# floe/backscrub

Measured on AMD Instinct MI355X. Metric: composited frames/sec at 640×480 (batch), 1/2/4/8 MI355X + mask IoU vs CPU ref, higher is better.
Workload: dtype f32 (network) / u8 (image kernels); 1 GPU; BASELINE configs[1]: batch=256 640x480 frames, segm_lite_v681.tflite; moving scene: ring of 4 batches, a new one every step; 1 step = prep+network+decode+mask+blend, inputs resident in HBM; streams_per_gpu=256, library=bsx 0.1 (HIP gfx950, f32 NHWC)

## Files before the change

backscrub_amd/csrc/gen_seg.cpp:

```cpp
#include "gen_seg.hpp"

#include <cstdarg>
#include <cstdio>

namespace bsx {
namespace {

const char kSegSource[] =
#include "seg_rtc_src.inc"
    ;

}

std::string seg_constants_text(const SegPlan& sp, const char* pre) {
  std::string out;
  auto P = [&](const char* fmt, ...) {
    char buf[1024];
    va_list ap;
    va_start(ap, fmt);
    vsnprintf(buf, sizeof buf, fmt, ap);
    va_end(ap);
    out += buf;
  };
  auto conv = [&](const char* n, const SegConvW& c) { P("  t.%s.w_off = %lldll; t.%s.b_off = %lldll; t.%s.Cin = %d; t.%s.Cout = %d; t.%s.cout_pad = %d; t.%s.act = %d;\n", n, c.w_off, n, c.b_off, n, c.Cin, n, c.Cout, n, c.cout_pad, n, c.act); };
  auto dw = [&](const char* n, const SegDwW& c) { P("  t.%s.w_off = %lldll; t.%s.b_off = %lldll; t.%s.C = %d; t.%s.act = %d;\n", n, c.w_off, n, c.b_off, n, c.C, n, c.act); };
  auto gate = [&](const char* n, const SegGate& g_) {
    P("  t.%s.n_parts = %d; t.%s.sum_parts = %d; t.%s.n_fc = %d; t.%s.timing_skip = %d;\n", n, g_.n_parts, n, g_.sum_parts, n, g_.n_fc, n, g_.timing_skip);
    for (int i = 0; i < 2; i++) {
      P("  t.%s.part[%d].off = %lldll; t.%s.part[%d].n = %d; t.%s.part[%d].C = %d; t.%s.part[%d].hw = (float)%.9g;\n", n, i, g_.part[i].off, n, i, g_.part[i].n, n, i, g_.part[i].C, n, i, (double)g_.part[i].hw);
      P("  t.%s.fc[%d].w_off = %lldll; t.%s.fc[%d].b_off = %lldll; t.%s.fc[%d].Cin = %d; t.%s.fc[%d].Cout = %d; t.%s.fc[%d].act = %d;\n", n, i, g_.fc[i].w_off, n, i, g_.fc[i].b_off, n, i, g_.fc[i].Cin, n, i,
              g_.fc[i].Cout, n, i, g_.fc[i].act);
    }
  };
  auto end = [&](int dbg_skip) { if (dbg_skip) P("  t.dbg_skip = %d;\n", dbg_skip); P("  return t; }();\n"); };
  const SegHead& H = sp.head; const SegK2& K2 = sp.k2; const SegK3& K3 = sp.k3; const SegTail& T = sp.tail;
  P("// segment descriptors of the loaded graph as constants (gen_seg.cpp: seg_constants_text)\nconstexpr SegHead %sHEAD = [] { SegHead t{};\n", pre);
  P("  t.H0 = %d; t.W0 = %d; t.H1 = %d; t.W1 = %d; t.H2 = %d; t.W2 = %d; t.stem_pt = %d; t.stem_pl = %d; t.dw_pt = %d; t.dw_pl = %d;\n", H.H0, H.W0, H.H1, H.W1, H.H2, H.W2, H.stem_pt, H.stem_pl, H.dw_pt, H.dw_pl);
  conv("stem", H.stem); conv("pw", H.pw); dw("dw", H.dw);
  P("  t.a_off = %lldll; t.b0_off = %lldll; t.part_a_off = %lldll; t.part_b0_off = %lldll; t.TR = %d; t.TC = %d; t.tiles_y = %d; t.tiles_x = %d; t.lds_floats = %d; t.rw = %d; t.m_ct = %uu;\n",
          H.a_off, H.b0_off, H.part_a_off, H.part_b0_off, H.TR, H.TC, H.tiles_y, H.tiles_x, H.lds_floats, H.rw, H.m_ct);
  end(H.dbg_skip);
  P("constexpr SegK2 %sK2 = [] { SegK2 t{};\n  t.H2 = %d; t.W2 = %d; t.H3 = %d; t.W3 = %d; t.dw_pt = %d; t.dw_pl = %d;\n", pre, K2.H2, K2.W2, K2.H3, K2.W3, K2.dw_pt, K2.dw_pl);
  gate("gate", K2.gate); conv("pw_a", K2.pw_a); conv("pw_b", K2.pw_b); dw("dw", K2.dw);
  P("  t.b0_off = %lldll; t.B_off = %lldll; t.c0_off = %lldll; t.part_B_off = %lldll; t.TR = %d; t.TC = %d; t.tiles_y = %d; t.tiles_x = %d; t.lds_floats = %d; t.rw = %d; t.m_ct = %uu;\n",
          K2.b0_off, K2.B_off, K2.c0_off, K2.part_B_off, K2.TR, K2.TC, K2.tiles_y, K2.tiles_x, K2.lds_floats, K2.rw, K2.m_ct);
  end(K2.dbg_skip);
  P("constexpr SegK3 %sK3 = [] { SegK3 t{};\n  t.H2 = %d; t.W2 = %d; t.HL = %d; t.WL = %d; t.half_pixel = %d; t.align_corners = %d;\n", pre, K3.H2, K3.W2, K3.HL, K3.WL, K3.half_pixel, K3.align_corners);
  conv("pw1", K3.pw1); conv("pw2", K3.pw2); dw("dw", K3.dw);
  P("  t.skip_off = %lldll; t.lo2_off = %lldll; t.g_off = %lldll; t.lo_off = %lldll; t.part_lo_off = %lldll; t.TR = %d; t.TC = %d; t.tiles_y = %d; t.tiles_x = %d; t.lds_floats = %d; t.lo_floats = %d; t.hs = (float)%.9g; t.ws = (float)%.9g;\n",
          K3.skip_off, K3.lo2_off, K3.g_off, K3.lo_off, K3.part_lo_off, K3.TR, K3.TC, K3.tiles_y, K3.tiles_x, K3.lds_floats, K3.lo_floats, (double)K3.hs, (double)K3.ws);
  end(K3.dbg_skip);
  P("constexpr SegTail %sTAIL = [] { SegTail t{};\n  t.H1 = %d; t.W1 = %d; t.HL = %d; t.WL = %d; t.H0 = %d; t.W0 = %d; t.half_pixel = %d; t.align_corners = %d;\n", pre, T.H1, T.W1, T.HL, T.WL, T.H0, T.W0, T.half_pixel, T.align_corners);
  gate("gate", T.gate); conv("pw", T.pw); dw("dw", T.dw);
  P("  t.tc_w_off = %lldll; t.tc_b_off = %lldll; t.Co = %d; t.act3 = %d; t.model_type = %d; t.skip_off = %lldll; t.lo_off = %lldll; t.pre_gate_off = %lldll; t.TR = %d; t.TC = %d; t.tiles_y = %d; t.tiles_x = %d; "
             "t.lds_floats = %d; t.lo_floats = %d; t.hs = (float)%.9g; t.ws = (float)%.9g;\n",
          T.tc_w_off, T.tc_b_off, T.Co, T.act3, T.model_type, T.skip_off, T.lo_off, T.pre_gate_off, T.TR, T.TC, T.tiles_y, T.tiles_x, T.lds_floats, T.lo_floats, (double)T.hs, (double)T.ws);
  end(T.dbg_skip);
  return out;
}

std::string generate_seg_source(const Plan& plan, bool h16, bool u8in, std::string* why) {
  auto fail = [&](const char* m) { if (why) *why = m; return std::string(); };
  if (!plan.seg.on) return fail("no segment kernels in this plan");
  const SegPlan& sp = plan.seg;
  const bool sig = sp.tail.act3 == kActSigmoid;
  if (!((sp.tail.Co == 2 && !sig) || sp.tail.Co == 1)) return fail("transpose-convolution output channels");
  std::string src = kSegSource;
  const std::string mark = "BSXS_SEG_CONSTANTS";
  const size_t at = src.find(mark);
  if (at == std::string::npos) return fail("embedded source has no constants marker");
  src.replace(at, mark.size(), seg_constants_text(sp, "kSeg"));
  char head[512];
  snprintf(head, sizeof head, "#define BSXS_SEG_RTC 1\n#define BSXS_SEG_HS %d\n#define BSXS_SEG_H16 %d\n#define BSXS_SEG_U8 %d\n#define BSXS_SEG_SIG %d\n#define BSXS_SEG_CO %d\n",
           sp.head.stem.act == kActHswish ? 1 : 0, h16 ? 1 : 0, u8in ? 1 : 0, sig ? 1 : 0, sp.tail.Co);
  return std::string(head) + src;
}

}
```

backscrub_amd/csrc/kernels_seg.hip:

```cpp
#ifndef __HIPCC_RTC__
#include <hip/hip_runtime.h>
#endif
#ifndef BSX_SEG_RTC
#include "debug_switches.hpp"

#include <algorithm>
#include <cstdlib>
#include <type_traits>

#include "kernels.hpp"
#include "mfma_tile.hpp"
#include "segments.hpp"
#endif

#if defined(BSX_SEG_RTC)
#define BSX_SEG_D(T, NAME) constexpr T d = kSeg##NAME; (void)d_rt
#elif defined(BSX_SEG_PROBE)
#define BSX_SEG_D(T, NAME) constexpr T d = kProbe##NAME; (void)d_rt
#else
#define BSX_SEG_D(T, NAME) const T& d = d_rt
#endif

namespace bsx {
#ifdef BSX_SEG_RTC
// ... 134 lines not shown
    fc(f2, s_hid, w2, b2, s_gate);
    __syncthreads();
  }
}

template <int SHR>
__device__ __forceinline__ float dpp_row_shr(float v) {
  return __builtin_bit_cast(float, __builtin_amdgcn_update_dpp(0, __builtin_bit_cast(int, v), 0x110 + SHR, 0xf, 0xf, true));
}
template <int MODE>
__device__ __forceinline__ void wave_reduce16(float4 v, float* s_red, int wave, int lane) {
  if (MODE == 0) {
    v.x += dpp_row_shr<1>(v.x); v.y += dpp_row_shr<1>(v.y); v.z += dpp_row_shr<1>(v.z); v.w += dpp_row_shr<1>(v.w);
    v.x += dpp_row_shr<2>(v.x); v.y += dpp_row_shr<2>(v.y); v.z += dpp_row_shr<2>(v.z); v.w += dpp_row_shr<2>(v.w);
    v.x += dpp_row_shr<4>(v.x); v.y += dpp_row_shr<4>(v.y); v.z += dpp_row_shr<4>(v.z); v.w += dpp_row_shr<4>(v.w);
    v.x += dpp_row_shr<8>(v.x); v.y += dpp_row_shr<8>(v.y); v.z += dpp_row_shr<8>(v.z); v.w += dpp_row_shr<8>(v.w);
    const int li = lane & 15;
    if (li >= 12) st4(s_red + (wave * 4 + (15 - li)) * 16 + 4 * (lane >> 4), li == 15 ? v : f4zero());
  } else {
    v.x += dpp_row_shr<4>(v.x); v.y += dpp_row_shr<4>(v.y); v.z += dpp_row_shr<4>(v.z); v.w += dpp_row_shr<4>(v.w);
    v.x += dpp_row_shr<8>(v.x); v.y += dpp_row_shr<8>(v.y); v.z += dpp_row_shr<8>(v.z); v.w += dpp_row_shr<8>(v.w);
    if ((lane & 12) == 12) st4(s_red + (wave * 4 + (lane >> 4)) * 16 + 4 * (lane & 3), v);
  }
}
__device__ __forceinline__ void store_partials(const float* s_red, float* dst ) {
  if (threadIdx.x < 16) {
    float s = 0.f;
#pragma unroll
    for (int j = 0; j < 16; j++) s += s_red[j * 16 + threadIdx.x];
    dst[threadIdx.x] = s;
  }
}

__device__ __forceinline__ void up_axis(int o, float scale, bool half_pixel, int in_size, int* lo, int* hi, float* frac) {
  const float v = half_pixel ? __fadd_rn(__fmul_rn((float)o + 0.5f, scale), -0.5f) : __fmul_rn((float)o, scale);
  const float fl = floorf(v);
  *lo = max((int)fl, 0);
  *hi = min((int)ceilf(v), in_size - 1);
  *frac = v - (float)*lo;
}
__device__ __forceinline__ float up_scale(int in, int out, bool align) { return (align && out > 1) ? (float)(in - 1) / (float)(out - 1) : (float)in / (float)out; }

__device__ __forceinline__ float quad_reduce_scatter(float p0, float p1, float p2, float p3, int quad) {
  const bool b0 = quad & 1, b1 = quad & 2;
  const float klo = (b0 ? p1 : p0) + dpp_quad(b0 ? p0 : p1, 1);
  const float khi = (b0 ? p3 : p2) + dpp_quad(b0 ? p2 : p3, 1);
  return (b1 ? khi : klo) + dpp_quad(b1 ? klo : khi, 2);
}

typedef float f4v __attribute__((ext_vector_type(4)));
__device__ __forceinline__ f4v ldv(const float* p) { return *reinterpret_cast<const f4v*>(p); }
__device__ __forceinline__ f4v tov(float4 a) { f4v r = {a.x, a.y, a.z, a.w}; return r; }
__device__ __forceinline__ float4 tof4(f4v a) { return make_float4(a.x, a.y, a.z, a.w); }
__device__ __forceinline__ f4v dw3x3(const float* __restrict__ zt, int RWF, int row0, const int (&co)[3], const f4v (&wd)[9]) {
  f4v acc = {0.f, 0.f, 0.f, 0.f};
  const float* base = zt + row0 * RWF;
#pragma unroll
  for (int fy = 0; fy < 3; fy++)
#pragma unroll
    for (int fx = 0; fx < 3; fx++) acc = __builtin_elementwise_fma(ldv(base + fy * RWF + co[fx]), wd[fy * 3 + fx], acc);
  return acc;
}

__device__ __forceinline__ uint32_t seg_meet_val(float l0, float l1) {
  const float d = l1 - l0;
  if (fabsf(l0) <= 80.f && fabsf(l1) <= 80.f && fabsf(d) >= 1e-4f) return d > 0.f ? 0u : 255u;
// ... 129 lines not shown
    const RowTile r0t = row_tile(t, ctiles, d.m_ct), r1t = row_tile(two ? t + 4 : t, ctiles, d.m_ct);
    const float* base0 = in_t + (2 * r0t.row) * rowf + 6 * min(16 * r0t.ct + li, AC - 1);
    const float* base1 = in_t + (2 * r1t.row) * rowf + 6 * min(16 * r1t.ct + li, AC - 1);
    float av0[7], av1[7];
#pragma unroll
    for (int s7 = 0; s7 < 7; s7++) { av0[s7] = base0[koff[s7]]; av1[s7] = base1[koff[s7]]; }
    f4acc acc0 = {0.f, 0.f, 0.f, 0.f}, acc1 = {0.f, 0.f, 0.f, 0.f};
#pragma unroll
    for (int s7 = 0; s7 < 7; s7++) {
      acc0 = __builtin_amdgcn_mfma_f32_16x16x4f32(ws[s7], av0[s7], acc0, 0, 0, 0);
      acc1 = __builtin_amdgcn_mfma_f32_16x16x4f32(ws[s7], av1[s7], acc1, 0, 0, 0);
    }
    stem_pw_epilogue(acc0, r0t);
    if (two) stem_pw_epilogue(acc1, r1t);
  }
  const int quad = lane & 3, px = lane >> 2;
  f4v wd[9];
#pragma unroll
  for (int k = 0; k < 9; k++) wd[k] = ldv(w + d.dw.w_off + k * 16 + 4 * quad);
  const f4v bias_d = ldv(w + d.dw.b_off + 4 * quad);
  const int cox[3] = {(2 * px) * 16 + 4 * quad, (2 * px + 1) * 16 + 4 * quad, (2 * px + 2) * 16 + 4 * quad};
  __syncthreads();

  float4 sumB = f4zero();
  for (int py = wave; py < d.TR && !(d.dbg_skip & 4); py += 4) {
    if (r0 + py >= d.H2) break;
    if (px < d.TC && c0 + px < d.W2) {
      const float4 v = clamp4(tof4(dw3x3(x_f, AC * 16, 2 * py, cox, wd) + bias_d), cl_dw);
      stg4<H16>(b0_out, (unsigned)(((r0 + py) * d.W2 + c0 + px) * 16 + 4 * quad), v);
      sumB = f4add(sumB, v);
    }
  }
  float* s_red = in_t;
  wave_reduce16<0>(sumA, s_red, wave, lane);
  wave_reduce16<1>(sumB, s_red + 256, wave, lane);
  __syncthreads();
  store_partials(s_red, fa + d.part_a_off + (long)t_ * 16);
  store_partials(s_red + 256, fa + d.part_b0_off + (long)t_ * 16);
}

#ifdef BSX_SEG_RTC
extern "C" __global__ __launch_bounds__(kSegThreads) __attribute__((amdgpu_waves_per_eu(6, 6))) void bsx_seg_k2(
#else
template <bool H16>
__global__ __launch_bounds__(kSegThreads) __attribute__((amdgpu_waves_per_eu(6, 6))) void seg_k2_k(
#endif
    const SegK2 d_rt, float* __restrict__ arena, long per_frame, const float* __restrict__ w, int n_frames) {
  BSX_SEG_D(SegK2, K2);
  unsigned f_, t_;
  xcd_frame_tile((unsigned)(d.tiles_y * d.tiles_x), (unsigned)n_frames, &f_, &t_);
  const int f = (int)f_, ty = (int)t_ / d.tiles_x, tx = (int)t_ - ty * d.tiles_x;
  const int r0 = ty * d.TR, c0 = tx * d.TC;
  const int BR = 2 * d.TR + 1, BC = 2 * d.TC + 1, br0 = 2 * r0 - d.dw_pt, bc0 = 2 * c0 - d.dw_pl, RW = d.rw, ctiles = RW >> 4;
  float* fa = arena + (size_t)f * (size_t)per_frame;
  float* B_t = seg_smem + kScrFloats;
  float* x_t = B_t + BR * RW * 16;
  const float* b0_in = fa + d.b0_off;
  float* B_out = fa + d.B_off;
  float* c0_out = fa + d.c0_off;
  const int tid = threadIdx.x, lane = tid & 63, wave = wave_uniform(tid >> 6), li = lane & 15, g = lane >> 4, cq4 = 4 * g;
  const int ntile = BR * ctiles, xe = li;
  const int la = col_a(li, g), lb = col_b(li, g, RW >> 1);
  constexpr int kB0 = 6;
  float4 b0v[kB0];
#pragma unroll
  for (int j = 0; j < kB0; j++) {
    const int t = wave + 4 * j;
    b0v[j] = f4zero();
    if (t < ntile) {
      const RowTile rt = row_tile(t, ctiles, d.m_ct);
      const int gy = br0 + rt.row, gx = bc0 + 16 * rt.ct + li;
      if (gy >= 0 && gy < d.H2 && gx >= 0 && gx < d.W2) b0v[j] = ldg4<H16>(b0_in, (unsigned)((gy * d.W2 + gx) * 16 + 4 * g));
    }
  }
  seg_gate(d.gate, fa, w, seg_smem, B_t);
  const float4 sv = ld4(seg_smem + kScrGate + 4 * g);
  float wr[4];
  load_wtile(wr, w, d.pw_a, 0, li, g);
  const float4 bias_a = ld4(w + d.pw_a.b_off + cq4);
  const Clamp cl_a = clamp_of(d.pw_a.act), cl_b = clamp_of(d.pw_b.act), cl_dw = clamp_of(d.dw.act);

  float4 sumB = f4zero();
#pragma unroll
  for (int j = 0; j < kB0; j++) {
    const int t = wave + 4 * j;
    if (t >= ntile) break;
    const RowTile rt = row_tile(t, ctiles, d.m_ct);
    float4 a = b0v[j];
    a = make_float4(__fmul_rn(a.x, sv.x), __fmul_rn(a.y, sv.y), __fmul_rn(a.z, sv.z), __fmul_rn(a.w, sv.w));
    const f4acc acc = mma16(a, wr);
    float4 v = acc_quad(acc);
    const int x2 = 16 * rt.ct + xe, hy = br0 + rt.row, hx = bc0 + x2;
    if (x2 < BC) {
      v = clamp4(f4add(v, bias_a), cl_a);
      st4(B_t + (rt.row * RW + 16 * rt.ct) * 16 + la, v);
      const bool row_owned = hy >= max(2 * r0, 0) && hy < min(2 * r0 + 2 * d.TR, d.H2);
      if (row_owned && hx >= 2 * c0 && hx < min(2 * c0 + 2 * d.TC, d.W2)) {
        stg4<H16>(B_out, (unsigned)((hy * d.W2 + hx) * 16 + cq4), v);
        sumB = f4add(sumB, v);
      }
    }
  }
  float* s_red = seg_smem + kScrRed;
  wave_reduce16<0>(sumB, s_red, wave, lane);
  __syncthreads();
  store_partials(s_red, fa + d.part_B_off + (long)t_ * 16);

  const int C = d.dw.C, ngrp = (C + 15) >> 4, quad = lane & 3, px = lane >> 2;
// ... 124 lines not shown
  float* z_t = seg_smem + kScrFloats;
  float* l_t = z_t + ZH * 256;
  float* lo_out = fa + d.lo_off;
  const int tid = threadIdx.x, lane = tid & 63, wave = wave_uniform(tid >> 6), li = lane & 15, g = lane >> 4, cq4 = 4 * g;
  const GatedPre pre = gated_prefetch<H16>(fa + d.skip_off, fa + d.lo2_off, d.H2, d.W2, d.HL, d.WL, d.half_pixel != 0, d.hs, d.ws, r0, c0, ZH, ZC, l_t);
  if (tid < 16) seg_smem[kScrGate + tid] = fa[d.g_off + tid];
  __syncthreads();
  gated_compute(pre, l_t, d.H2, d.W2, d.HL, d.WL, d.half_pixel != 0, d.hs, d.ws, seg_smem + kScrGate, d.pw1, w, r0, c0, ZH, ZC, z_t);
  const int pc = min(li, 13);
  const int coz[3] = {col_a(pc, g), col_a(pc + 1, g), col_a(pc + 2, g)};
  f4v wd[9];
#pragma unroll
  for (int k = 0; k < 9; k++) wd[k] = ldv(w + d.dw.w_off + k * 16 + cq4);
  const f4v bias_d = ldv(w + d.dw.b_off + cq4);
  const Clamp cl_dw = clamp_of(d.dw.act), cl_2 = clamp_of(d.pw2.act);
  float wr[4];
  load_wtile(wr, w, d.pw2, 0, li, g);
  const float4 bias2 = ld4(w + d.pw2.b_off + cq4);
  __syncthreads();
  float4 sum = f4zero();
  const int xe = li;
  for (int py = wave; py < d.TR && r0 + py < d.H2; py += 4) {
    const f4v zc = ldv(z_t + (py + 1) * 256 + coz[1]);
    const float4 dv = clamp4(tof4(dw3x3(z_t, 256, py, coz, wd) + bias_d), cl_dw);
    const f4acc acc = mma16(f4add(dv, tof4(zc)), wr);
    float4 v = acc_quad(acc);
    if (xe < d.TC && c0 + xe < d.W2) {
      v = clamp4(f4add(v, bias2), cl_2);
      stg4<H16>(lo_out, (unsigned)(((r0 + py) * d.W2 + c0 + xe) * 16 + cq4), v);
      sum = f4add(sum, v);
    }
  }
  float* s_red = seg_smem + kScrRed;
  wave_reduce16<0>(sum, s_red, wave, lane);
  __syncthreads();
  store_partials(s_red, fa + d.part_lo_off + (long)t_ * 16);
}

#ifdef BSX_SEG_RTC
extern "C" __global__ __launch_bounds__(kSegThreads) __attribute__((amdgpu_waves_per_eu(5, 5))) void bsx_seg_tail(
#else
template <int CO, bool LOGITS, bool SIGMOID, bool H16>
__global__ __launch_bounds__(kSegThreads) __attribute__((amdgpu_waves_per_eu(5, 5))) void seg_tail_k(
#endif
    const SegTail d_rt, float* __restrict__ arena, long per_frame, float* __restrict__ net_out,
                                                          uint8_t* __restrict__ ofinal, const float* __restrict__ w, int n_frames, const int* __restrict__ slot_of) {
  BSX_SEG_D(SegTail, TAIL);
  unsigned f_, t_;
  xcd_frame_tile((unsigned)(d.tiles_y * d.tiles_x), (unsigned)n_frames, &f_, &t_);
  const int f = (int)f_, ty = (int)t_ / d.tiles_x, tx = (int)t_ - ty * d.tiles_x;
  const int r0 = ty * d.TR, c0 = tx * d.TC, ZH = d.TR + 2, ZC = d.TC + 2;
  float* fa = arena + (size_t)f * (size_t)per_frame;
  float* z_t = seg_smem + kScrFloats;
  float* l_t = z_t + max(ZH * 256, kGateStageFloats);
  uint8_t* of = ofinal + (size_t)(slot_of ? slot_of[f] : f) * (size_t)(d.H0 * d.W0);
  float* no = net_out + (size_t)f * (size_t)(d.H0 * d.W0 * CO);
  const int tid = threadIdx.x, lane = tid & 63, wave = wave_uniform(tid >> 6), li = lane & 15, g = lane >> 4, cq4 = 4 * g;
  const int fy = g >> 1, fx = g & 1, ix = c0 + li;
  const GatedPre pre = gated_prefetch<H16>(fa + d.skip_off, fa + d.lo_off, d.H1, d.W1, d.HL, d.WL, d.half_pixel != 0, d.hs, d.ws, r0, c0, ZH, ZC, l_t);
  constexpr int kRowsB = 5;
  const bool lane_on = li < d.TC && ix < d.W1;
  uint8_t prev[kRowsB];
  if (!LOGITS) {
#pragma unroll
    for (int j = 0; j < kRowsB; j++) {
      const int py = wave + 4 * j, iy = r0 + py;
      prev[j] = 0;
      if (py < d.TR && iy < d.H1 && lane_on) prev[j] = of[(unsigned)((2 * iy + fy) * d.W0 + 2 * ix + fx)];
    }
  }
  if (d.pre_gate_off >= 0) {
    if (tid < 16) seg_smem[kScrGate + tid] = fa[d.pre_gate_off + tid];
    __syncthreads();
  } else seg_gate(d.gate, fa, w, seg_smem, z_t);
  if (!(d.dbg_skip & 1)) gated_compute(pre, l_t, d.H1, d.W1, d.HL, d.WL, d.half_pixel != 0, d.hs, d.ws, seg_smem + kScrGate, d.pw, w, r0, c0, ZH, ZC, z_t);
  if (d.dbg_skip & 2) return;
  f4v wd[9];
#pragma unroll
  for (int k = 0; k < 9; k++) wd[k] = ldv(w + d.dw.w_off + k * 16 + cq4);
  const f4v bias_d = ldv(w + d.dw.b_off + cq4);
  float wtr[4];
#pragma unroll
  for (int r = 0; r < 4; r++) wtr[r] = (li & 3) < CO ? w[d.tc_w_off + (unsigned)((((li >> 2) * CO + (li & 3)) * 16) + cq4 + r)] : 0.f;
  float bt[CO];
#pragma unroll
  for (int oc = 0; oc < CO; oc++) bt[oc] = w[d.tc_b_off + oc];
  const Clamp cl_dw = clamp_of(d.dw.act);
  const int pc = min(li, 13);
  const int coz[3] = {col_a(pc, g), col_a(pc + 1, g), col_a(pc + 2, g)};
  __syncthreads();
#pragma unroll
  for (int j = 0; j < kRowsB; j++) {
    const int py = wave + 4 * j, iy = r0 + py;
    if (py >= d.TR || iy >= d.H1) break;
    const f4v zc = ldv(z_t + (py + 1) * 256 + coz[1]);
    const float4 t4 = f4add(clamp4(tof4(dw3x3(z_t, 256, py, coz, wd) + bias_d), cl_dw), tof4(zc));
    const f4acc acc = mma16(t4, wtr);
    if (lane_on) {
      float o[CO];
#pragma unroll
      for (int oc = 0; oc < CO; oc++) {
        o[oc] = bt[oc] + acc[oc];
        if (SIGMOID) o[oc] = sigmoid1(o[oc]);
      }
      const int oy = 2 * iy + fy, ox = 2 * ix + fx;
      const unsigned opix = (unsigned)(oy * d.W0 + ox);
      if (LOGITS) {
// ... 96 lines not shown
```

backscrub_amd/csrc/plan.cpp:

```cpp
#include "debug_switches.hpp"
#include "plan.hpp"
#include "gen_seg.hpp"
#include "gen_mid.hpp"

#include <algorithm>
#include <cmath>
#include <cstdio>
#include <cstdlib>
#include <cstring>
#include <map>

namespace bsx {
namespace {

void conv_geometry(int in, int k, int s, int d, bool same, int* out, int* pad) {
  int eff = (k - 1) * d + 1;
  *out = same ? (in + s - 1) / s : (in + s - eff) / s;
  int total = (*out - 1) * s + eff - in;
  *pad = total > 0 ? total / 2 : 0;
}

uint16_t f32_to_f16_rn(float f) {
  uint32_t x; memcpy(&x, &f, 4);
  const uint32_t sign = (x >> 16) & 0x8000u;
// ... 589 lines not shown
  h.lds_floats = seg_head_lds_floats(h);
  h.rw = seg_row_width(2 * h.TC + 1); h.m_ct = (65536u + (unsigned)(h.rw / 16) - 1) / (unsigned)(h.rw / 16);
  if (h.TR > 4 || h.TC > 15 || (4 * h.TC + 3) * 3 > 192) return seg_fail(30);
  SegK2& k2 = sp.k2;
  k2.H2 = hdw.OH; k2.W2 = hdw.OW; k2.H3 = kdw.OH; k2.W3 = kdw.OW; k2.dw_pt = kdw.pad_t; k2.dw_pl = kdw.pad_l;
  k2.pw_a = conv_w(pwa); k2.pw_b = conv_w(pwb); k2.dw = dw_w(kdw);
  split(k2.H3, tgt[2], &k2.TR, &k2.tiles_y); split(k2.W3, tgt[3], &k2.TC, &k2.tiles_x);
  k2.lds_floats = seg_k2_lds_floats(k2);
  k2.rw = seg_row_width(2 * k2.TC + 1); k2.m_ct = (65536u + (unsigned)(k2.rw / 16) - 1) / (unsigned)(k2.rw / 16);
  if (k2.TC > 15 || ((2 * k2.TR + 1) * (k2.rw / 16) + 3) / 4 > 6) return seg_fail(31);
  SegK3& k3 = sp.k3;
  k3.H2 = kp1.OH; k3.W2 = kp1.OW; k3.HL = kr.H; k3.WL = kr.W; k3.half_pixel = kr.half_pixel; k3.align_corners = kr.align_corners;
  k3.pw1 = conv_w(kp1); k3.pw2 = conv_w(kp2); k3.dw = dw_w(kd);
  split(k3.H2, tgt[4], &k3.TR, &k3.tiles_y); split(k3.W2, tgt[5], &k3.TC, &k3.tiles_x);
  k3.hs = seg_up_scale(k3.HL, k3.H2, k3.align_corners != 0); k3.ws = seg_up_scale(k3.WL, k3.W2, k3.align_corners != 0);
  if (!BSX_DBG_ENV("BSX_SEG_LO_WORST")) k3.lo_floats = seg_lo_window_floats(k3.H2, k3.W2, k3.HL, k3.WL, k3.half_pixel != 0, k3.align_corners != 0, k3.TR, k3.TC, k3.tiles_y, k3.tiles_x);
  k3.lds_floats = seg_k3_lds_floats(k3);
  if (k3.TC > 14 || k3.TR > 18) return seg_fail(32);
  SegTail& tl = sp.tail;
  tl.H1 = tpw.OH; tl.W1 = tpw.OW; tl.HL = tr.H; tl.WL = tr.W; tl.H0 = ttc.OH; tl.W0 = ttc.OW; tl.half_pixel = tr.half_pixel; tl.align_corners = tr.align_corners;
  tl.pw = conv_w(tpw); tl.dw = dw_w(tdw); tl.tc_w_off = (long long)ttc.w_off; tl.tc_b_off = (long long)ttc.b_off; tl.Co = ttc.Cout; tl.act3 = ttc.act;
  split(tl.H1, tgt[6], &tl.TR, &tl.tiles_y); split(tl.W1, tgt[7], &tl.TC, &tl.tiles_x);
  tl.hs = seg_up_scale(tl.HL, tl.H1, tl.align_corners != 0); tl.ws = seg_up_scale(tl.WL, tl.W1, tl.align_corners != 0);
  if (!BSX_DBG_ENV("BSX_SEG_LO_WORST")) tl.lo_floats = seg_lo_window_floats(tl.H1, tl.W1, tl.HL, tl.WL, tl.half_pixel != 0, tl.align_corners != 0, tl.TR, tl.TC, tl.tiles_y, tl.tiles_x);
  tl.lds_floats = seg_tail_lds_floats(tl);
  if (tl.TC > 14 || tl.TR > 18) return seg_fail(33);
  const int lds_cap = 160 * 256;
  if (h.lds_floats > lds_cap || k2.lds_floats > lds_cap || k3.lds_floats > lds_cap || tl.lds_floats > lds_cap) return seg_fail(24);
  if (ttc.OH != 2 * tpw.OH || ttc.OW != 2 * tpw.OW || h.H2 != k3.H2 || h.W2 != k3.W2) return seg_fail(25);
  if (h.tiles_y * h.tiles_x > 1024 || k2.tiles_y * k2.tiles_x > 1024 || k3.tiles_y * k3.tiles_x > 1024) return seg_fail(26);

  const int pA = synth("partials(A)", h.tiles_y * h.tiles_x, 16), pb0 = synth("partials(b0)", h.tiles_y * h.tiles_x, 16);
  const int pB = synth("partials(B)", k2.tiles_y * k2.tiles_x, 16), plo = synth("partials(lo)", k3.tiles_y * k3.tiles_x, 16);
  const int pgt = BSX_DBG_ENV("BSX_SEG_NO_GATE_KERNEL") ? -1 : synth("gate(tail)", 1, 16);
  if (pgt >= 0) plan->tensor_off[pgt] = reserve(16);
  for (int t : {A, b0, B, c0, lo2, lo, kf2.out, pA, pb0, pB, plo}) plan->tensor_off[t] = reserve(g.tensors[t].elems());
  for (int t : {hpw.out, g1.out, f1a.out, f1b.out, pwb.out, up2, kg.out, kf1.out, kp1.out, kd.out, up, tg.out, tf1.out, tf2.out, tpw.out, tdw.out})
    if (t != g.output) plan->tensor_off[t] = -1;
  plan->arena_floats_per_stream = top;
  plan->seg_stored = {A, b0, B, c0, lo};

  h.a_off = plan->tensor_off[A]; h.b0_off = plan->tensor_off[b0]; h.part_a_off = plan->tensor_off[pA]; h.part_b0_off = plan->tensor_off[pb0];
  k2.b0_off = plan->tensor_off[b0]; k2.B_off = plan->tensor_off[B]; k2.c0_off = plan->tensor_off[c0]; k2.part_B_off = plan->tensor_off[pB];
  k2.gate.n_parts = 1; k2.gate.n_fc = 2; k2.gate.sum_parts = 0;
  k2.gate.part[0].off = plan->tensor_off[pb0]; k2.gate.part[0].n = h.tiles_y * h.tiles_x; k2.gate.part[0].C = 16; k2.gate.part[0].hw = (float)(h.H2 * h.W2);
  k2.gate.fc[0] = fc_w(f1a); k2.gate.fc[1] = fc_w(f1b);
  k3.skip_off = plan->tensor_off[B]; k3.lo2_off = plan->tensor_off[lo2]; k3.g_off = plan->tensor_off[kf2.out]; k3.lo_off = plan->tensor_off[lo];
  k3.part_lo_off = plan->tensor_off[plo];
  tl.skip_off = plan->tensor_off[A]; tl.lo_off = plan->tensor_off[lo];
  tl.gate.n_parts = 2; tl.gate.n_fc = 2; tl.gate.sum_parts = tg.gap_sum ? 1 : 0;
  tl.gate.part[0].off = plan->tensor_off[pA]; tl.gate.part[0].n = h.tiles_y * h.tiles_x; tl.gate.part[0].C = 16; tl.gate.part[0].hw = (float)(h.H1 * h.W1);
  tl.gate.part[1].off = plan->tensor_off[plo]; tl.gate.part[1].n = k3.tiles_y * k3.tiles_x; tl.gate.part[1].C = 16; tl.gate.part[1].hw = (float)(k3.H2 * k3.W2);
  tl.gate.fc[0] = fc_w(tf1); tl.gate.fc[1] = fc_w(tf2);
  if (BSX_DBG_ENV("BSX_SEG_GATE_SKIP")) k2.gate.timing_skip = tl.gate.timing_skip = 1;
  if (const char* e = BSX_DBG_ENV("BSX_SEG_SKIP")) sscanf(e, "%d,%d,%d,%d", &h.dbg_skip, &k2.dbg_skip, &k3.dbg_skip, &tl.dbg_skip);
  tl.pre_gate_off = pgt >= 0 ? plan->tensor_off[pgt] : -1;
  if (tl.gate.fc[0].Cin != (tl.gate.sum_parts ? 16 : 32) || k2.gate.fc[0].Cin != 16) return seg_fail(27);

  std::vector<Step> mid(S.begin() + 9, S.begin() + (NS - 14));
  Step gate = kg;
  gate.concat_in = {B, lo2};
  gate.in0 = B;
  gate.label += "*";
  mid.push_back(gate); mid.push_back(kf1); mid.push_back(kf2);
  std::map<int, int> part_n, part_hw;
  part_n[B] = k2.tiles_y * k2.tiles_x; part_hw[B] = k2.H2 * k2.W2;
  const long B_real = plan->tensor_off[B];
  plan->tensor_off[B] = plan->tensor_off[pB];
  build_frame_program(g, plan, mid, {c0, B, lo2, kf2.out}, part_n, part_hw);
  plan->tensor_off[B] = B_real;
  if (plan->program.empty()) return seg_fail(28);
  sp.on = true;
  plan->seg = sp;
#ifdef BSX_DEBUG_SWITCHES
  if (const char* path = BSX_DBG_ENV("BSX_SEG_DUMP")) {
    if (FILE* f = fopen(path, "w")) { fputs(seg_constants_text(sp, "kProbe").c_str(), f); fclose(f); }
  }
#endif
  char line[256];
  plan->seg_text.clear();
  auto add = [&](const char* name, int TR, int TC, int ty, int tx, int lds, std::initializer_list<int> stores) {
    snprintf(line, sizeof line, "segment %-5s tile %dx%d, %dx%d tiles per frame, LDS %.1f KiB, stores", name, TR, TC, ty, tx, lds / 256.0);
    plan->seg_text += line;
    for (int t : stores) plan->seg_text += " t" + std::to_string(t);
    plan->seg_text += stores.size() ? "\n" : " the network output\n";
  };
  add("head", h.TR, h.TC, h.tiles_y, h.tiles_x, h.lds_floats, {A, b0}); add("k2", k2.TR, k2.TC, k2.tiles_y, k2.tiles_x, k2.lds_floats, {B, c0});
  add("k3", k3.TR, k3.TC, k3.tiles_y, k3.tiles_x, k3.lds_floats, {lo}); add("tail", tl.TR, tl.TC, tl.tiles_y, tl.tiles_x, tl.lds_floats, {});
  return true;
}


MidGeometry mid_geometry_default() {
  static const MidGeometry geo = [] {
    MidGeometry m{kFrameThreads, kLdsTotalFloats};
    if (const char* e = BSX_DBG_ENV("BSX_MID_LANES")) { const int v = atoi(e); if (v == 512 || v == 1024) m.lanes = v; }
    if (const char* e = BSX_DBG_ENV("BSX_MID_LDS_KB")) { const int v = atoi(e); if (v >= 64 && v <= 160) m.lds_floats = v * 256; }
    return m;
  }();
  return geo;
}

bool build_plan(const Graph& g_in, Plan* plan, std::string* err, bool reuse_arena, bool segments) {
  auto fail = [&](const std::string& m) { if (err) *err = m; return false; };
  { const MidGeometry geo = mid_geometry_default(); plan->mid_lanes = geo.lanes; plan->lds_total_floats = geo.lds_floats; }
  Graph g = g_in;
  int NT = (int)g.tensors.size();
  const int NN = (int)g.nodes.size();

  std::vector<std::vector<int>> users(NT);
  for (int i = 0; i < NN; i++) for (int t : g.nodes[i].inputs) if (t >= 0 && !g.tensors[t].is_const) users[t].push_back(i);
  auto single_user = [&](int t) -> int { return (t != g.output && users[t].size() == 1) ? users[t][0] : -1; };

  std::vector<char> fused(NN, 0);
  std::vector<Step> steps;
  std::vector<float>& W = plan->weights;
  W.clear();
  auto align_w = [&]() { while (W.size() % 4) W.push_back(0.f); };

  for (int i = 0; i < NN; i++) {
    if (fused[i]) continue;
// ... 511 lines not shown
```

backscrub_amd/csrc/segments.hpp:

```cpp
#pragma once
#ifndef BSX_SEG_RTC
#include <algorithm>
#include <cmath>
#include <cstdint>
#endif

namespace bsx {

struct SegConvW { long long w_off = 0, b_off = 0; int Cin = 0, Cout = 0, cout_pad = 0, act = 0; };
struct SegDwW { long long w_off = 0, b_off = 0; int C = 0, act = 0; };
struct SegFc { long long w_off = 0, b_off = 0; int Cin = 0, Cout = 0, act = 0; };
struct SegPart { long long off = 0; int n = 0, C = 0; float hw = 1.f; };
struct SegGate {
  int n_parts = 0, sum_parts = 0, n_fc = 0;
  int timing_skip = 0;
  SegPart part[2];
  SegFc fc[2];
};

constexpr int kSegThreads = 256;
constexpr int kSegMaxC = 16;

struct SegHead {
  int H0 = 0, W0 = 0, H1 = 0, W1 = 0, H2 = 0, W2 = 0;
  int stem_pt = 0, stem_pl = 0, dw_pt = 0, dw_pl = 0;
  SegConvW stem, pw;
  SegDwW dw;
  long long a_off = 0, b0_off = 0, part_a_off = 0, part_b0_off = 0;
  int TR = 0, TC = 0, tiles_y = 0, tiles_x = 0;
  int lds_floats = 0;
  int dbg_skip = 0;
  int rw = 0;
  unsigned m_ct = 0;
};

struct SegK2 {
  int H2 = 0, W2 = 0, H3 = 0, W3 = 0;
  int dw_pt = 0, dw_pl = 0;
  SegGate gate;
  SegConvW pw_a, pw_b;
  SegDwW dw;
  long long b0_off = 0, B_off = 0, c0_off = 0, part_B_off = 0;
  int TR = 0, TC = 0, tiles_y = 0, tiles_x = 0;
  int lds_floats = 0;
  int dbg_skip = 0;
  int rw = 0;
  unsigned m_ct = 0;
};

struct SegK3 {
  int H2 = 0, W2 = 0, HL = 0, WL = 0;
  int half_pixel = 0, align_corners = 0;
  SegConvW pw1, pw2;
  SegDwW dw;
  long long skip_off = 0, lo2_off = 0, g_off = 0, lo_off = 0, part_lo_off = 0;
  int TR = 0, TC = 0, tiles_y = 0, tiles_x = 0;
  int lds_floats = 0;
  int lo_floats = 0;
  float hs = 0.f, ws = 0.f;
  int dbg_skip = 0;
};

struct SegTail {
  int H1 = 0, W1 = 0, HL = 0, WL = 0, H0 = 0, W0 = 0;
  int half_pixel = 0, align_corners = 0;
  SegGate gate;
  SegConvW pw;
  SegDwW dw;
  long long tc_w_off = 0, tc_b_off = 0;
  int Co = 0, act3 = 0, model_type = 0;
  long long skip_off = 0, lo_off = 0;
  long long pre_gate_off = -1;
  int TR = 0, TC = 0, tiles_y = 0, tiles_x = 0;
  int lds_floats = 0;
  int lo_floats = 0;
  float hs = 0.f, ws = 0.f;
  int dbg_skip = 0;
};

constexpr int kSegLoStride = 16;
constexpr int kSegLoTileFloats = 12 * 16 * kSegLoStride;
constexpr int kSegScratchFloats = 640;
constexpr int kSegGateStageFloats = 512 + 2 * (32 * 32 + 32);
#ifndef BSX_SEG_RTC
inline int seg_row_width(int cols) { return (cols + 15) / 16 * 16; }
inline int seg_head_lds_floats(const SegHead& d) {
  const int AR = 2 * d.TR + 1, AC = 2 * d.TC + 1, IR = 2 * AR + 1, IC = 2 * AC + 1;
  const int win = (IR * IC * 3 + 3) & ~3;
// ... 42 lines not shown
```

Baseline: 727,300 frames/s.

## Compute tail gate from per-tile FC1 contributions instead of separate gate kernel

Head and k3 kernels now multiply each tile's pooled channel partials by the first gate FC weights and store per-tile FC1 contributions. The tail kernel sums these linear contributions, applies the activation, and runs FC2 in one wave, so the separate gate kernel and the per-tile pooled gate recomputation are no longer needed. The tail issues this request early so its loads overlap the prefetch. In exchange, head and k3 do extra DPP reductions and FC1 stores, and the arena grows. A debug gate-dump path is also added.

After: 732,600 frames/s (median of 6 runs). Within noise of the previous version (+0.7%).

```diff
diff --git a/backscrub_amd/csrc/gen_seg.cpp b/backscrub_amd/csrc/gen_seg.cpp
--- a/backscrub_amd/csrc/gen_seg.cpp
+++ b/backscrub_amd/csrc/gen_seg.cpp
@@ -26,12 +26,15 @@
   auto dw = [&](const char* n, const SegDwW& c) { P("  t.%s.w_off = %lldll; t.%s.b_off = %lldll; t.%s.C = %d; t.%s.act = %d;\n", n, c.w_off, n, c.b_off, n, c.C, n, c.act); };
   auto gate = [&](const char* n, const SegGate& g_) {
     P("  t.%s.n_parts = %d; t.%s.sum_parts = %d; t.%s.n_fc = %d; t.%s.timing_skip = %d;\n", n, g_.n_parts, n, g_.sum_parts, n, g_.n_fc, n, g_.timing_skip);
+    P("  t.%s.from_fc1 = %d; t.%s.fc1_off[0] = %lldll; t.%s.fc1_off[1] = %lldll;\n", n, g_.from_fc1, n, g_.fc1_off[0], n, g_.fc1_off[1]);
+    if (g_.dump_off >= 0) P("  t.%s.dump_off = %lldll;\n", n, g_.dump_off);
     for (int i = 0; i < 2; i++) {
       P("  t.%s.part[%d].off = %lldll; t.%s.part[%d].n = %d; t.%s.part[%d].C = %d; t.%s.part[%d].hw = (float)%.9g;\n", n, i, g_.part[i].off, n, i, g_.part[i].n, n, i, g_.part[i].C, n, i, (double)g_.part[i].hw);
       P("  t.%s.fc[%d].w_off = %lldll; t.%s.fc[%d].b_off = %lldll; t.%s.fc[%d].Cin = %d; t.%s.fc[%d].Cout = %d; t.%s.fc[%d].act = %d;\n", n, i, g_.fc[i].w_off, n, i, g_.fc[i].b_off, n, i, g_.fc[i].Cin, n, i,
               g_.fc[i].Cout, n, i, g_.fc[i].act);
     }
   };
+  auto fc1 = [&](const char* n, const SegFc1& c) { P("  t.%s.off = %lldll; t.%s.w_off = %lldll; t.%s.C1 = %d; t.%s.Cin = %d; t.%s.col = %d;\n", n, c.off, n, c.w_off, n, c.C1, n, c.Cin, n, c.col); };
   auto end = [&](int dbg_skip) { if (dbg_skip) P("  t.dbg_skip = %d;\n", dbg_skip); P("  return t; }();\n"); };
   const SegHead& H = sp.head; const SegK2& K2 = sp.k2; const SegK3& K3 = sp.k3; const SegTail& T = sp.tail;
   P("// segment descriptors of the loaded graph as constants (gen_seg.cpp: seg_constants_text)\nconstexpr SegHead %sHEAD = [] { SegHead t{};\n", pre);
@@ -39,6 +42,7 @@
   conv("stem", H.stem); conv("pw", H.pw); dw("dw", H.dw);
   P("  t.a_off = %lldll; t.b0_off = %lldll; t.part_a_off = %lldll; t.part_b0_off = %lldll; t.TR = %d; t.TC = %d; t.tiles_y = %d; t.tiles_x = %d; t.lds_floats = %d; t.rw = %d; t.m_ct = %uu;\n",
           H.a_off, H.b0_off, H.part_a_off, H.part_b0_off, H.TR, H.TC, H.tiles_y, H.tiles_x, H.lds_floats, H.rw, H.m_ct);
+  fc1("fc1_a", H.fc1_a);
   end(H.dbg_skip);
   P("constexpr SegK2 %sK2 = [] { SegK2 t{};\n  t.H2 = %d; t.W2 = %d; t.H3 = %d; t.W3 = %d; t.dw_pt = %d; t.dw_pl = %d;\n", pre, K2.H2, K2.W2, K2.H3, K2.W3, K2.dw_pt, K2.dw_pl);
   gate("gate", K2.gate); conv("pw_a", K2.pw_a); conv("pw_b", K2.pw_b); dw("dw", K2.dw);
@@ -49,6 +53,7 @@
   conv("pw1", K3.pw1); conv("pw2", K3.pw2); dw("dw", K3.dw);
   P("  t.skip_off = %lldll; t.lo2_off = %lldll; t.g_off = %lldll; t.lo_off = %lldll; t.part_lo_off = %lldll; t.TR = %d; t.TC = %d; t.tiles_y = %d; t.tiles_x = %d; t.lds_floats = %d; t.lo_floats = %d; t.hs = (float)%.9g; t.ws = (float)%.9g;\n",
           K3.skip_off, K3.lo2_off, K3.g_off, K3.lo_off, K3.part_lo_off, K3.TR, K3.TC, K3.tiles_y, K3.tiles_x, K3.lds_floats, K3.lo_floats, (double)K3.hs, (double)K3.ws);
+  fc1("fc1_lo", K3.fc1_lo);
   end(K3.dbg_skip);
   P("constexpr SegTail %sTAIL = [] { SegTail t{};\n  t.H1 = %d; t.W1 = %d; t.HL = %d; t.WL = %d; t.H0 = %d; t.W0 = %d; t.half_pixel = %d; t.align_corners = %d;\n", pre, T.H1, T.W1, T.HL, T.WL, T.H0, T.W0, T.half_pixel, T.align_corners);
   gate("gate", T.gate); conv("pw", T.pw); dw("dw", T.dw);
diff --git a/backscrub_amd/csrc/kernels_seg.hip b/backscrub_amd/csrc/kernels_seg.hip
--- a/backscrub_amd/csrc/kernels_seg.hip
+++ b/backscrub_amd/csrc/kernels_seg.hip
@@ -190,6 +190,87 @@
   }
 }
 
+constexpr int kFc1Regs = 8;
+__device__ __forceinline__ void fc1_weights(const SegFc1& c, const float* __restrict__ w, float (&wv)[kFc1Regs]) {
+  unsigned t = threadIdx.x;
+  asm volatile("" : "+v"(t));
+  const int ch = t & 15, r = (t >> 4) & 3;
+  const float* w1 = w + c.w_off;
+#pragma unroll
+  for (int k = 0; k < kFc1Regs; k++) {
+    const int o = r + 4 * k;
+    wv[k] = (c.off >= 0 && o < c.C1) ? w1[(unsigned)(o * c.Cin + c.col + ch)] : 0.f;
+  }
+}
+__device__ __forceinline__ void store_partials_fc1(const float* s_red, float* part, const SegFc1& c, const float (&wv)[kFc1Regs], float* fc1) {
+  unsigned t = threadIdx.x;
+  asm volatile("" : "+v"(t));
+  const int ch = t & 15, r = t >> 4;
+  float s = 0.f;
+#pragma unroll
+  for (int j = 0; j < 16; j++) s += s_red[j * 16 + ch];
+  if (t < 16) part[t] = s;
+  if (c.off < 0) return;
+#pragma unroll
+  for (int k = 0; k < kFc1Regs; k++) {
+    const int o = r + 4 * k;
+    if (4 * k >= c.C1) break;
+    float p = __fmul_rn(wv[k], s);
+    p += dpp_row_shr<1>(p); p += dpp_row_shr<2>(p); p += dpp_row_shr<4>(p); p += dpp_row_shr<8>(p);
+    if (ch == 15 && o < c.C1) fc1[o] = p;
+  }
+}
+
+constexpr int kGateLd = 5;
+struct GateReq { float v[2][kGateLd]; float b1, b2, w2[8]; };
+__device__ __forceinline__ int gate_c1p(int C1) { return C1 <= 8 ? 8 : (C1 <= 16 ? 16 : 32); }
+__device__ __forceinline__ float lane_read(float v, int src) { return __builtin_bit_cast(float, __builtin_amdgcn_ds_bpermute(src << 2, __builtin_bit_cast(int, v))); }
+__device__ __forceinline__ GateReq gate_fc1_request(const SegGate& gt, const float* __restrict__ fa, const float* __restrict__ w) {
+  const int lane = threadIdx.x & 63, C1 = gt.fc[0].Cout, C1p = gate_c1p(C1), c = lane & (C1p - 1), sl = lane / C1p, nsl = 64 / C1p;
+  GateReq q;
+#pragma unroll
+  for (int k = 0; k < 2; k++)
+#pragma unroll
+    for (int j = 0; j < kGateLd; j++) {
+      const int i = sl + j * nsl;
+      q.v[k][j] = (k < gt.n_parts && i < gt.part[k].n && c < C1) ? (fa + gt.fc1_off[k])[(unsigned)(i * C1 + c)] : 0.f;
+    }
+  q.b1 = c < C1 ? (w + gt.fc[0].b_off)[(unsigned)c] : 0.f;
+  const int out = lane >> 2, ks = lane & 3, kper = C1p >> 2;
+#pragma unroll
+  for (int j = 0; j < 8; j++) {
+    const int idx = ks * kper + j;
+    q.w2[j] = (j < kper && idx < C1) ? (w + gt.fc[1].w_off)[(unsigned)(out * C1 + idx)] : 0.f;
+  }
+  q.b2 = (w + gt.fc[1].b_off)[(unsigned)out];
+  return q;
+}
+__device__ __forceinline__ void gate_fc1_finish(const SegGate& gt, const GateReq& q, const float* __restrict__ fa, float* s_gate) {
+  const int lane = threadIdx.x & 63, C1 = gt.fc[0].Cout, C1p = gate_c1p(C1), c = lane & (C1p - 1), sl = lane / C1p, nsl = 64 / C1p;
+  float h = 0.f;
+#pragma unroll
+  for (int k = 0; k < 2; k++) {
+    if (k >= gt.n_parts) break;
+    float a = 0.f;
+#pragma unroll
+    for (int j = 0; j < kGateLd; j++) a += q.v[k][j];
+    for (int i = sl + kGateLd * nsl; i < gt.part[k].n; i += nsl) a += c < C1 ? (fa + gt.fc1_off[k])[(unsigned)(i * C1 + c)] : 0.f;
+    for (int m = C1p; m < 64; m <<= 1) a += lane_read(a, lane ^ m);
+    h += a / gt.part[k].hw;
+  }
+  h = sg_act(h + q.b1, gt.fc[0].act);
+  const int out = lane >> 2, ks = lane & 3, kper = C1p >> 2;
+  float acc = 0.f;
+#pragma unroll
+  for (int j = 0; j < 8; j++) {
+    if (j >= kper) break;
+    acc = fmaf(lane_read(h, ks * kper + j), q.w2[j], acc);
+  }
+  acc += dpp_quad(acc, 1);
+  acc += dpp_quad(acc, 2);
+  if (ks == 0) s_gate[out] = sg_act(acc + q.b2, gt.fc[1].act);
+}
+
 __device__ __forceinline__ void up_axis(int o, float scale, bool half_pixel, int in_size, int* lo, int* hi, float* frac) {
   const float v = half_pixel ? __fadd_rn(__fmul_rn((float)o + 0.5f, scale), -0.5f) : __fmul_rn((float)o, scale);
   const float fl = floorf(v);
@@ -385,10 +466,12 @@
     }
   }
   float* s_red = in_t;
+  float wfa[kFc1Regs];
+  if (wave == 0) fc1_weights(d.fc1_a, w, wfa);
   wave_reduce16<0>(sumA, s_red, wave, lane);
   wave_reduce16<1>(sumB, s_red + 256, wave, lane);
   __syncthreads();
-  store_partials(s_red, fa + d.part_a_off + (long)t_ * 16);
+  if (wave == 0) store_partials_fc1(s_red, fa + d.part_a_off + (long)t_ * 16, d.fc1_a, wfa, fa + d.fc1_a.off + (long)t_ * d.fc1_a.C1);
   store_partials(s_red + 256, fa + d.part_b0_off + (long)t_ * 16);
 }
 
@@ -427,6 +510,7 @@
     }
   }
   seg_gate(d.gate, fa, w, seg_smem, B_t);
+  if (d.gate.dump_off >= 0 && t_ == 0 && tid < 16) fa[d.gate.dump_off + tid] = seg_smem[kScrGate + tid];
   const float4 sv = ld4(seg_smem + kScrGate + 4 * g);
   float wr[4];
   load_wtile(wr, w, d.pw_a, 0, li, g);
@@ -617,9 +701,11 @@
     }
   }
   float* s_red = seg_smem + kScrRed;
+  float wfl[kFc1Regs];
+  if (wave == 0) fc1_weights(d.fc1_lo, w, wfl);
   wave_reduce16<0>(sum, s_red, wave, lane);
   __syncthreads();
-  store_partials(s_red, fa + d.part_lo_off + (long)t_ * 16);
+  if (wave == 0) store_partials_fc1(s_red, fa + d.part_lo_off + (long)t_ * 16, d.fc1_lo, wfl, fa + d.fc1_lo.off + (long)t_ * d.fc1_lo.C1);
 }
 
 #ifdef BSX_SEG_RTC
@@ -642,6 +728,9 @@
   float* no = net_out + (size_t)f * (size_t)(d.H0 * d.W0 * CO);
   const int tid = threadIdx.x, lane = tid & 63, wave = wave_uniform(tid >> 6), li = lane & 15, g = lane >> 4, cq4 = 4 * g;
   const int fy = g >> 1, fx = g & 1, ix = c0 + li;
+  const bool gate_fc1 = d.gate.from_fc1 && !d.gate.timing_skip;
+  GateReq gq = {};
+  if (gate_fc1 && wave == 0) gq = gate_fc1_request(d.gate, fa, w);
   const GatedPre pre = gated_prefetch<H16>(fa + d.skip_off, fa + d.lo_off, d.H1, d.W1, d.HL, d.WL, d.half_pixel != 0, d.hs, d.ws, r0, c0, ZH, ZC, l_t);
   constexpr int kRowsB = 5;
   const bool lane_on = li < d.TC && ix < d.W1;
@@ -654,10 +743,14 @@
       if (py < d.TR && iy < d.H1 && lane_on) prev[j] = of[(unsigned)((2 * iy + fy) * d.W0 + 2 * ix + fx)];
     }
   }
-  if (d.pre_gate_off >= 0) {
+  if (gate_fc1) {
+    if (wave == 0) gate_fc1_finish(d.gate, gq, fa, seg_smem + kScrGate);
+    __syncthreads();
+  } else if (d.pre_gate_off >= 0) {
     if (tid < 16) seg_smem[kScrGate + tid] = fa[d.pre_gate_off + tid];
     __syncthreads();
   } else seg_gate(d.gate, fa, w, seg_smem, z_t);
+  if (d.gate.dump_off >= 0 && t_ == 0 && tid < 16) fa[d.gate.dump_off + tid] = seg_smem[kScrGate + tid];
   if (!(d.dbg_skip & 1)) gated_compute(pre, l_t, d.H1, d.W1, d.HL, d.WL, d.half_pixel != 0, d.hs, d.ws, seg_smem + kScrGate, d.pw, w, r0, c0, ZH, ZC, z_t);
   if (d.dbg_skip & 2) return;
   f4v wd[9];
diff --git a/backscrub_amd/csrc/plan.cpp b/backscrub_amd/csrc/plan.cpp
--- a/backscrub_amd/csrc/plan.cpp
+++ b/backscrub_amd/csrc/plan.cpp
@@ -645,11 +645,17 @@
 
   const int pA = synth("partials(A)", h.tiles_y * h.tiles_x, 16), pb0 = synth("partials(b0)", h.tiles_y * h.tiles_x, 16);
   const int pB = synth("partials(B)", k2.tiles_y * k2.tiles_x, 16), plo = synth("partials(lo)", k3.tiles_y * k3.tiles_x, 16);
-  const int pgt = BSX_DBG_ENV("BSX_SEG_NO_GATE_KERNEL") ? -1 : synth("gate(tail)", 1, 16);
+  const bool fc1_route = !BSX_DBG_ENV("BSX_SEG_GATE_KERNEL") && !BSX_DBG_ENV("BSX_SEG_NO_GATE_KERNEL") && !BSX_DBG_ENV("BSX_SEG_GATE_SKIP");
+  const int pgt = (fc1_route || BSX_DBG_ENV("BSX_SEG_NO_GATE_KERNEL")) ? -1 : synth("gate(tail)", 1, 16);
   if (pgt >= 0) plan->tensor_off[pgt] = reserve(16);
+  const int c1_tail = tf1.Cout;
+  const int qA = fc1_route ? synth("fc1(A)", h.tiles_y * h.tiles_x, c1_tail) : -1, qlo = fc1_route ? synth("fc1(lo)", k3.tiles_y * k3.tiles_x, c1_tail) : -1;
+  for (int t : {qA, qlo}) if (t >= 0) plan->tensor_off[t] = reserve(g.tensors[t].elems());
   for (int t : {A, b0, B, c0, lo2, lo, kf2.out, pA, pb0, pB, plo}) plan->tensor_off[t] = reserve(g.tensors[t].elems());
   for (int t : {hpw.out, g1.out, f1a.out, f1b.out, pwb.out, up2, kg.out, kf1.out, kp1.out, kd.out, up, tg.out, tf1.out, tf2.out, tpw.out, tdw.out})
     if (t != g.output) plan->tensor_off[t] = -1;
+  const bool gate_dump = BSX_DBG_ENV("BSX_SEG_GATE_DUMP") != nullptr;
+  if (gate_dump) for (int t : {f1b.out, tf2.out}) plan->tensor_off[t] = reserve(16);
   plan->arena_floats_per_stream = top;
   plan->seg_stored = {A, b0, B, c0, lo};
 
@@ -666,6 +672,14 @@
   tl.gate.part[1].off = plan->tensor_off[plo]; tl.gate.part[1].n = k3.tiles_y * k3.tiles_x; tl.gate.part[1].C = 16; tl.gate.part[1].hw = (float)(k3.H2 * k3.W2);
   tl.gate.fc[0] = fc_w(tf1); tl.gate.fc[1] = fc_w(tf2);
   if (BSX_DBG_ENV("BSX_SEG_GATE_SKIP")) k2.gate.timing_skip = tl.gate.timing_skip = 1;
+  if (fc1_route) {
+    const SegFc& t1 = tl.gate.fc[0];
+    h.fc1_a = SegFc1{plan->tensor_off[qA], t1.w_off, t1.Cout, t1.Cin, 0};
+    k3.fc1_lo = SegFc1{plan->tensor_off[qlo], t1.w_off, t1.Cout, t1.Cin, tl.gate.sum_parts ? 0 : 16};
+    tl.gate.from_fc1 = 1;
+    tl.gate.fc1_off[0] = h.fc1_a.off; tl.gate.fc1_off[1] = k3.fc1_lo.off;
+  }
+  if (gate_dump) { k2.gate.dump_off = plan->tensor_off[f1b.out]; tl.gate.dump_off = plan->tensor_off[tf2.out]; plan->seg_stored.push_back(f1b.out); plan->seg_stored.push_back(tf2.out); }
   if (const char* e = BSX_DBG_ENV("BSX_SEG_SKIP")) sscanf(e, "%d,%d,%d,%d", &h.dbg_skip, &k2.dbg_skip, &k3.dbg_skip, &tl.dbg_skip);
   tl.pre_gate_off = pgt >= 0 ? plan->tensor_off[pgt] : -1;
   if (tl.gate.fc[0].Cin != (tl.gate.sum_parts ? 16 : 32) || k2.gate.fc[0].Cin != 16) return seg_fail(27);
@@ -700,6 +714,13 @@
   };
   add("head", h.TR, h.TC, h.tiles_y, h.tiles_x, h.lds_floats, {A, b0}); add("k2", k2.TR, k2.TC, k2.tiles_y, k2.tiles_x, k2.lds_floats, {B, c0});
   add("k3", k3.TR, k3.TC, k3.tiles_y, k3.tiles_x, k3.lds_floats, {lo}); add("tail", tl.TR, tl.TC, tl.tiles_y, tl.tiles_x, tl.lds_floats, {});
+  snprintf(line, sizeof line, "gates: k2 t%d, tail t%d%s\n", f1b.out, tf2.out, gate_dump ? " (stored by tile 0)" : "");
+  plan->seg_text += line;
+  if (fc1_route) {
+    snprintf(line, sizeof line, "tail gate from per-tile FC1 contributions: fc1(A) %dx%d @%lld, fc1(lo) %dx%d @%lld\n", h.tiles_y * h.tiles_x, c1_tail, h.fc1_a.off,
+             k3.tiles_y * k3.tiles_x, c1_tail, k3.fc1_lo.off);
+    plan->seg_text += line;
+  }
   return true;
 }
 
diff --git a/backscrub_amd/csrc/segments.hpp b/backscrub_amd/csrc/segments.hpp
--- a/backscrub_amd/csrc/segments.hpp
+++ b/backscrub_amd/csrc/segments.hpp
@@ -14,9 +14,14 @@
 struct SegGate {
   int n_parts = 0, sum_parts = 0, n_fc = 0;
   int timing_skip = 0;
+  int from_fc1 = 0;
+  long long fc1_off[2] = {-1, -1};
+  long long dump_off = -1;
   SegPart part[2];
   SegFc fc[2];
 };
+
+struct SegFc1 { long long off = -1, w_off = 0; int C1 = 0, Cin = 0, col = 0; };
 
 constexpr int kSegThreads = 256;
 constexpr int kSegMaxC = 16;
@@ -27,6 +32,7 @@
   SegConvW stem, pw;
   SegDwW dw;
   long long a_off = 0, b0_off = 0, part_a_off = 0, part_b0_off = 0;
+  SegFc1 fc1_a;
   int TR = 0, TC = 0, tiles_y = 0, tiles_x = 0;
   int lds_floats = 0;
   int dbg_skip = 0;
@@ -54,6 +60,7 @@
   SegConvW pw1, pw2;
   SegDwW dw;
   long long skip_off = 0, lo2_off = 0, g_off = 0, lo_off = 0, part_lo_off = 0;
+  SegFc1 fc1_lo;
   int TR = 0, TC = 0, tiles_y = 0, tiles_x = 0;
   int lds_floats = 0;
   int lo_floats = 0;
```
